# caumente/multi_task_breast_cancer

Hardware: AMD Instinct MI355X
Metric: training images/sec (1-ch 256x256, U-Net++ MT) (higher is better)
Workload: dtype bf16; 1 GPU; MTUNetPlusPlus seg+cls deep-supervision step (Dice+Focal, alpha=0.5, Adam eps 1e-4), per-GPU batch 32, 1x256x256, bf16 MFMA operands (3x3 convs, ConvT) and 16-bit stored conv outputs / activations; fp32 accumulation, gradient sums, statistics, losses, parameters and optimizer, random-init weights (BASELINE.json configs[1]); global_batch=32, parallelism=dp1

## Files before the change

include/mtbc.h:

```cpp
#ifndef MTBC_H
#define MTBC_H

#include <stddef.h>
#include <stdint.h>

#ifdef __cplusplus
extern "C" {
#endif

#define MTBC_VERSION 203
#define MTBC_MAX_SEGS 6
#define MTBC_STEM_MAX_CIN 5

enum {
    MTBC_OK = 0,
    MTBC_E_BADSHAPE = -1,
    MTBC_E_BADARG = -2,
    MTBC_E_WORKSPACE = -3,
    MTBC_E_LAUNCH = -4,
    MTBC_E_UNSUPPORTED = -5
};

int mtbc_version(void);
const char* mtbc_strerror(int code);
// ... 186 lines not shown
    float* y;
    const float* dy;
    float* dx;       int64_t dx_batch_stride;
    int32_t accumulate_dx;
    float* dw;       float* dbias;
    int32_t accumulate_dw;
    void* workspace; size_t workspace_bytes;
    int32_t x_layout;
    int32_t x_type;
} mtbc_conv1x1_args;

size_t mtbc_conv1x1_wgrad_workspace(const mtbc_conv1x1_args* a);
int mtbc_conv1x1_fwd(const mtbc_conv1x1_args* a, void* stream);
int mtbc_conv1x1_dgrad(const mtbc_conv1x1_args* a, void* stream);
int mtbc_conv1x1_wgrad(const mtbc_conv1x1_args* a, void* stream);

typedef struct {
    int32_t N, C, H, W;
    const float* x;  float* y;
    const float* dy; float* dx;
} mtbc_gap_args;
int mtbc_gap_fwd(const mtbc_gap_args* a, void* stream);
int mtbc_gap_bwd(const mtbc_gap_args* a, void* stream);

typedef struct {
    int32_t N, In, Out, relu;
    const float* x; const float* w; const float* bias; float* y;
    const float* dy; float* dx;
    float* dw; float* dbias; int32_t accumulate_dw;
    void* workspace; size_t workspace_bytes;
// ... 219 lines not shown
```

multi_task_breast_cancer_amd/_lib.py:

```python
from __future__ import annotations

import ctypes as C
import os
from typing import Optional

_HERE = os.path.dirname(os.path.abspath(__file__))
LIB_PATH = os.environ.get("MTBC_LIB") or os.path.join(_HERE, "libmtbc_hip.so")

MAX_SEGS = 6
STEM_MAX_CIN = 5
c_float_p = C.POINTER(C.c_float)


class MtbcError(RuntimeError):
    pass


LAYOUT_PLANAR, LAYOUT_C8 = 0, 1


class Seg(C.Structure):
    _fields_ = [("ptr", C.c_void_p), ("batch_stride", C.c_int64), ("channels", C.c_int32), ("accumulate", C.c_int32)]


# ... 225 lines not shown
    _fields_ = [("w", C.c_void_p), ("packed", C.c_void_p), ("Cin", C.c_int32), ("Cout", C.c_int32),
                ("kind", C.c_int32), ("compute", C.c_int32)]


class WViewDesc(C.Structure):
    _fields_ = [("w", C.c_void_p), ("dst", C.c_void_p), ("Cout", C.c_int32), ("Cin", C.c_int32), ("ci_off", C.c_int32),
                ("ci_cnt", C.c_int32), ("mode", C.c_int32), ("k_off", C.c_int32), ("K", C.c_int32)]


EXPORTS = [
    "mtbc_version", "mtbc_strerror", "mtbc_arch",
    "mtbc_conv3x3_packed_elems", "mtbc_conv3x3_packed_dgrad_elems", "mtbc_conv3x3_pack_fwd",
    "mtbc_conv3x3_pack_dgrad", "mtbc_conv3x3_packed_lp_elems", "mtbc_conv3x3_pack_lp", "mtbc_conv3x3_pack_many", "mtbc_c8_pack", "mtbc_c8_unpack", "mtbc_c8_pack16", "mtbc_conv3x3_weight_view", "mtbc_conv3x3_weight_view_many", "mtbc_augment_flip_rotate", "mtbc_convT_head_combine", "mtbc_convT_head_expand", "mtbc_conv3x3_wgrad_workspace", "mtbc_conv3x3_wgrad_sync_bytes", "mtbc_conv3x3_stats_slots", "mtbc_conv3x3_kernel_name", "mtbc_conv3x3_fwd", "mtbc_conv3x3_dgrad",
    "mtbc_conv3x3_wgrad", "mtbc_instnorm_fwd_workspace", "mtbc_instnorm_coop_state_bytes", "mtbc_instnorm_coop_error_offset", "mtbc_instnorm_c8_supported", "mtbc_instnorm_bwd_team", "mtbc_instnorm_dparam_many", "mtbc_instnorm_kernel_name", "mtbc_instnorm_lrelu_fwd", "mtbc_instnorm_lrelu_bwd", "mtbc_maxpool2_fwd",
    "mtbc_maxpool2_bwd", "mtbc_convT_wgrad_workspace", "mtbc_convT_fwd_c8_supported", "mtbc_convT_fwd", "mtbc_convT_dgrad", "mtbc_convT_wgrad",
    "mtbc_conv1x1_wgrad_workspace", "mtbc_conv1x1_fwd", "mtbc_conv1x1_dgrad", "mtbc_conv1x1_wgrad",
    "mtbc_gap_fwd", "mtbc_gap_bwd", "mtbc_linear_fwd", "mtbc_linear_bwd", "mtbc_dice_fwd", "mtbc_dice_bwd",
    "mtbc_focal_fwd_bwd", "mtbc_loss_mix", "mtbc_loss_scale_begin", "mtbc_loss_scale_check",
    "mtbc_loss_scale_update_host", "mtbc_loss_scale_begin_host", "mtbc_optim_step", "mtbc_optim_dynamic", "mtbc_loss_scale_optim", "mtbc_optim_step_host",
    "mtbc_dice_counts", "mtbc_program_run",
    "mtbc_program_run_ms", "mtbc_event_create", "mtbc_event_destroy",
    "mtbc_seg_metrics_workspace_size", "mtbc_seg_metrics", "mtbc_batch_assemble", "mtbc_train_metrics",
    "mtbc_eval_metrics",
]

ABI_VERSION = 203
_lib: Optional[C.CDLL] = None


def load() -> C.CDLL:
    global _lib
# ... 60 lines not shown
                      ("mtbc_conv1x1_wgrad", Conv1x1Args), ("mtbc_gap_fwd", GapArgs), ("mtbc_gap_bwd", GapArgs),
                      ("mtbc_linear_fwd", LinearArgs), ("mtbc_linear_bwd", LinearArgs),
                      ("mtbc_dice_fwd", DiceArgs), ("mtbc_dice_bwd", DiceArgs), ("mtbc_focal_fwd_bwd", FocalArgs)):
        getattr(lib, name).restype = C.c_int
        getattr(lib, name).argtypes = [C.POINTER(typ), C.c_void_p]
    lib.mtbc_instnorm_coop_state_bytes.restype = C.c_size_t
    lib.mtbc_instnorm_coop_state_bytes.argtypes = []
    lib.mtbc_instnorm_coop_error_offset.restype = C.c_size_t
    lib.mtbc_instnorm_coop_error_offset.argtypes = []
    lib.mtbc_instnorm_bwd_team.restype = C.c_int32
    lib.mtbc_instnorm_bwd_team.argtypes = [C.POINTER(InstNormArgs)]
    lib.mtbc_instnorm_dparam_many.restype = C.c_int
    lib.mtbc_instnorm_dparam_many.argtypes = [C.POINTER(DparamDesc), C.c_int32, C.c_void_p]
    lib.mtbc_instnorm_c8_supported.restype = C.c_int
    lib.mtbc_instnorm_c8_supported.argtypes = [C.POINTER(InstNormArgs), C.c_int32]
    lib.mtbc_convT_fwd_c8_supported.restype = C.c_int
    lib.mtbc_convT_fwd_c8_supported.argtypes = [C.POINTER(ConvTArgs)]
    lib.mtbc_loss_mix.restype = C.c_int
    lib.mtbc_loss_mix.argtypes = [C.c_void_p, C.c_void_p, C.c_float, C.c_void_p, C.c_void_p]
    lib.mtbc_dice_counts.restype = C.c_int
    lib.mtbc_dice_counts.argtypes = [C.c_void_p, C.c_void_p, C.c_int64, C.c_void_p, C.c_void_p]
    for name in ("mtbc_loss_scale_begin", "mtbc_loss_scale_check"):
        getattr(lib, name).restype = C.c_int
        getattr(lib, name).argtypes = [C.POINTER(LossScaleArgs), C.c_void_p]
    for name in ("mtbc_loss_scale_update_host", "mtbc_loss_scale_begin_host"):
        getattr(lib, name).restype = C.c_int
        getattr(lib, name).argtypes = [C.POINTER(LossScaleArgs)]
    lib.mtbc_optim_step.restype = C.c_int
    lib.mtbc_optim_step.argtypes = [C.POINTER(OptimArgs), C.c_void_p]
    lib.mtbc_optim_dynamic.restype = C.c_int
# ... 43 lines not shown
```

multi_task_breast_cancer_amd/csrc/common.h:

```cpp
#pragma once
#include <hip/hip_runtime.h>
#include <stdint.h>
#include <stdlib.h>
#include "../../include/mtbc.h"

#define MTBC_WAVE 64

typedef float f32x4 __attribute__((ext_vector_type(4)));

#define MTBC_CHECK_LAUNCH()                                   \
    do {                                                      \
        hipError_t e__ = hipGetLastError();                   \
        if (e__ != hipSuccess) return MTBC_E_LAUNCH;          \
    } while (0)

#ifdef MTBC_PROBES
#include <stdlib.h>
static inline int mtbc_probe_int(const char* name, int dflt) { const char* v = getenv(name); return v ? atoi(v) : dflt; }
static inline bool mtbc_probe_set(const char* name) { return getenv(name) != nullptr; }
#define MTBC_DBG_BIT(p, bit) ((p).dbg & (bit))
#else
#define mtbc_probe_int(name, dflt) (dflt)
#define mtbc_probe_set(name) (false)
#define MTBC_DBG_BIT(p, bit) (0)
// ... 113 lines not shown
    NK_STATS_FIN, NK_APPLY_FWD, NK_BSTATS_FIN, NK_APPLY_BWD,
    NK_R1_FIN, NK_DPARAM,
    NK_FWD_REG, NK_CHUNK_STATS, NK_CHUNK_APPLY, NK_FWD_STREAM, NK_BWD, NK_BWD_REG
};
struct NormLaunch { int k; int t[6]; int threads; int T, rounds; };
struct NormChoice {
    static constexpr int MAX = 4;
    int n; NormLaunch l[MAX];
    void add(int k, int t0 = 0, int t1 = 0, int t2 = 0, int t3 = 0, int t4 = 0, int t5 = 0) { if (n == MAX) abort(); l[n++] = NormLaunch{k, {t0, t1, t2, t3, t4, t5}, 0, 0, 0}; }
    void add(const NormLaunch& k) { if (n == MAX) abort(); l[n++] = k; }
    NormLaunch& last() { return l[n - 1]; }
};
extern "C" int mtbc_i_instnorm_fwd_c8(const mtbc_instnorm_args* a, hipStream_t st, NormChoice* query);
extern "C" int mtbc_i_instnorm_bwd_c8(const mtbc_instnorm_args* a, float* part, hipStream_t st, NormChoice* query);
extern "C" int mtbc_i_instnorm_bwd_c8_team(const mtbc_instnorm_args* a);
int mtbc_i_maxpool_c8_fwd(const mtbc_maxpool_args* a, hipStream_t st);
int mtbc_i_maxpool_c8_bwd(const mtbc_maxpool_args* a, hipStream_t st);
int mtbc_i_conv1x1_c8_fwd(const mtbc_conv1x1_args* a, hipStream_t st);
size_t mtbc_i_conv1x1_c8_wgrad_workspace(const mtbc_conv1x1_args* a);
int mtbc_i_conv1x1_c8_wgrad(const mtbc_conv1x1_args* a, hipStream_t st);
int mtbc_i_splitk_reduce(const float* partial, float* out, int nsplit, size_t elems, int accumulate, hipStream_t st);
int mtbc_i_splitk_reduce2(const float* partial, float* out, float* out2, int nsplit, size_t elems1, size_t elems2, int accumulate, hipStream_t st);
bool mtbc_i_convT2_fwd_ok(const mtbc_convT_args* a);
int mtbc_i_convT2_fwd(const mtbc_convT_args* a, hipStream_t st);
bool mtbc_i_convT2_fwd_c8_ok(const mtbc_convT_args* a);
int mtbc_i_convT2_fwd_c8(const mtbc_convT_args* a, hipStream_t st);
bool mtbc_i_convT2_fwd_lp_c8_ok(const mtbc_convT_args* a);
int mtbc_i_convT2_fwd_lp_c8(const mtbc_convT_args* a, hipStream_t st);
bool mtbc_i_convT2_dgrad_ok(const mtbc_convT_args* a);
bool mtbc_i_convT2_wgrad_ok(const mtbc_convT_args* a);
// ... 8 lines not shown
```

multi_task_breast_cancer_amd/csrc/norm_coop.hip:

```cpp
#include "common.h"
#include <stddef.h>
#include <type_traits>

namespace {

constexpr int CO_THREADS = 512, CO_WAVES = CO_THREADS / 64;
constexpr int CO_MAXT = 128, CO_NV = 16;
constexpr unsigned CO_SPIN_MAX = 1u << 26;
constexpr size_t CO_MAILBOX_OFF = 256;
constexpr int CO_MAX_TEAMS = 1024;
constexpr size_t CO_TEAM_WORDS = 2 * CO_MAXT * CO_NV;
struct CoopHdr { unsigned epoch, done, err, pad; };

struct CoP {
    int N, C, HW, G8, T, items, nteams, f16;
    float eps, slope;
    const float* z; const float* gamma; const float* beta;
    float* y; long long ybs;
    unsigned short* y8;
    float* mean; float* rstd;
    const float* dy; long long dybs;
    unsigned short* dz8;
    float* part;
    float* part3;
// ... 560 lines not shown
#pragma unroll
            for (int c = 0; c < 8; ++c) yb[(size_t)c * p.HW + px] = v[c];
        }
        if (yh) {
            if (k == 1) {
#pragma unroll
                for (int c = 0; c < 8; ++c) {
                    const unsigned lo = (okeep[c >> 1] >> (16 * (c & 1))) & 0xffffu, hi = (o[c >> 1] >> (16 * (c & 1))) & 0xffffu;
                    *reinterpret_cast<unsigned*>(yh + (size_t)c * p.HW + px - 1) = lo | (hi << 16);
                }
            } else okeep = o;
        }
    }
}

__global__ void in_bstats_finalize_kernel(const float* __restrict__ part, int slots, int C, int HW, float* __restrict__ m12,
                                          float* __restrict__ dparam_part, int planes) {
    const int plane = blockIdx.x * (blockDim.x >> 6) + (threadIdx.x >> 6), lane = threadIdx.x & 63;
    if (plane >= planes) return;
    const int n = plane / C, c = plane % C;
    const float* q = part + ((size_t)n * slots * C + c) * 2;
    double s1 = 0.0, s2 = 0.0;
    for (int t = lane; t < slots; t += 64) { const float2 v = *reinterpret_cast<const float2*>(q + (size_t)t * C * 2); s1 += (double)v.x; s2 += (double)v.y; }
    s1 = wave_sum_d(s1); s2 = wave_sum_d(s2);
    if (lane == 0) {
        m12[2 * plane] = (float)(s1 / (double)HW); m12[2 * plane + 1] = (float)(s2 / (double)HW);
        if (dparam_part) { dparam_part[3 * plane] = (float)s1; dparam_part[3 * plane + 1] = (float)s2; dparam_part[3 * plane + 2] = 0.f; }
    }
}
template <bool F16, bool ZF16>
// ... 245 lines not shown
        pl = plan_team<false>(p.items, p.HW, var_of(a), a->coop_reserve_cus);
        if (!pl.ok) return MTBC_E_UNSUPPORTED;
        choose_c8(&ch, false, p.HW, p.items, var_of(a), &pl);
    }
    if (query) { for (int i = 0; i < ch.n; ++i) query->add(ch.l[i]); return MTBC_OK; }
    for (int i = 0; i < ch.n; ++i) {
        const NormLaunch& k = ch.l[i];
        if (k.k == NK_STATS_FIN) hipLaunchKernelGGL(in_stats_finalize_kernel, dim3(cdiv(planes, 4)), dim3(256), 0, st, a->stats_partial, a->stats_slots, a->C, p.HW, a->eps, a->mean, a->rstd, planes);
        else if (k.k == NK_APPLY_FWD) launch_apply_fwd(k, g, st, p, a->stats_partial, a->stats_slots);
        else launch_chosen_c8<false>(k, p, pl, st);
        MTBC_CHECK_LAUNCH();
    }
    return MTBC_OK;
}

int mtbc_i_instnorm_bwd_c8_team(const mtbc_instnorm_args* a) {
    if (!a || a->N <= 0 || a->C <= 0 || a->C % 8) return 0;
    if (a->H * a->W <= SOLO_MAX_HW) return 1;
    const CoPlan pl = plan_team<true>(a->N * (a->C / 8), a->H * a->W, var_of(a), a->coop_reserve_cus);
    return pl.ok ? pl.T : 0;
}
int mtbc_i_instnorm_bwd_c8(const mtbc_instnorm_args* a, float* part, hipStream_t st, NormChoice* query) {
    CoP p; int rc = fill_coop(a, &p); if (rc) return rc;
    if ((!p.z && !p.z8) || (!p.dy && !p.r1 && !p.pg) || !p.dz8 || !p.mean || !p.rstd || (reinterpret_cast<uintptr_t>(p.dz8) & 15)) return MTBC_E_BADARG;
    if (!p.dy && a->dy_layout == MTBC_LAYOUT_C8) return MTBC_E_BADARG;
    if ((p.r1 || p.pg) && a->stats_partial) return MTBC_E_UNSUPPORTED;
    if (a->dy_layout == MTBC_LAYOUT_C8) {
        if ((reinterpret_cast<uintptr_t>(a->dy) & 15) || a->dy_batch_stride % 8 || a->n_dy_extra < 0 || a->n_dy_extra > 1) return MTBC_E_BADARG;
        p.dy8 = reinterpret_cast<const unsigned short*>(a->dy); p.dy8bs = a->dy_batch_stride; p.dy = nullptr;
        if (a->n_dy_extra == 1) { if (!a->dy_extra[0]) return MTBC_E_BADARG; p.dyx = a->dy_extra[0]; }
// ... 47 lines not shown
```

multi_task_breast_cancer_amd/csrc/program.hip:

```cpp
#include "common.h"

extern "C" {

int mtbc_version(void) { return MTBC_VERSION; }
const char* mtbc_arch(void) { return "gfx950"; }

const char* mtbc_strerror(int code) {
    switch (code) {
        case MTBC_OK: return "ok";
        case MTBC_E_BADSHAPE: return "bad shape";
        case MTBC_E_BADARG: return "bad argument (null or misaligned pointer)";
        case MTBC_E_WORKSPACE: return "workspace missing or too small";
        case MTBC_E_LAUNCH: return "kernel launch failed";
        case MTBC_E_UNSUPPORTED: return "unsupported configuration";
        default: return "unknown error";
    }
}

static inline bool is_pack(int32_t k) { return k == MTBC_OP_CONV3_PACK_FWD || k == MTBC_OP_CONV3_PACK_DGRAD || k == MTBC_OP_CONV3_PACK_LP; }

int mtbc_event_create(void** event) {
    if (!event) return MTBC_E_BADARG;
    hipEvent_t e;
    if (hipEventCreateWithFlags(&e, hipEventDisableTiming) != hipSuccess) return MTBC_E_LAUNCH;
// ... 66 lines not shown
        if (o->kind == MTBC_OP_IN_DPARAM) {
            mtbc_dparam_desc d[64];
            int32_t n = 0;
            while (n < 64 && i + n < first + count && ops[i + n].kind == MTBC_OP_IN_DPARAM) { d[n] = ops[i + n].u.dparam; ++n; }
            rc = mtbc_instnorm_dparam_many(d, n, stream);
            if (rc != MTBC_OK) { if (failed_index) *failed_index = i; return rc; }
            i += n - 1;
            continue;
        }
        if (o->kind == MTBC_OP_CONVT_WGRAD && i + 1 < first + count && ops[i + 1].kind == MTBC_OP_CONVT_DGRAD) {
            bool fused = false;
            rc = mtbc_i_convT_bwd_pair(&o->u.convT, &ops[i + 1].u.convT, stream, &fused);
            if (rc != MTBC_OK) { if (failed_index) *failed_index = i; return rc; }
            if (fused) { ++i; continue; }
        }
        switch (o->kind) {
            case MTBC_OP_CONV3_FWD: rc = mtbc_conv3x3_fwd(&o->u.conv3, stream); break;
            case MTBC_OP_CONV3_DGRAD: rc = mtbc_conv3x3_dgrad(&o->u.conv3, stream); break;
            case MTBC_OP_CONV3_WGRAD: rc = mtbc_conv3x3_wgrad(&o->u.conv3, stream); break;
            case MTBC_OP_CONV3_PACK_FWD: rc = mtbc_conv3x3_pack_fwd(o->u.pack.w, o->u.pack.packed, o->u.pack.Cin, o->u.pack.Cout, stream); break;
            case MTBC_OP_CONV3_PACK_DGRAD: rc = mtbc_conv3x3_pack_dgrad(o->u.pack.w, o->u.pack.packed, o->u.pack.Cin, o->u.pack.Cout, stream); break;
            case MTBC_OP_HEAD_COMBINE: rc = mtbc_convT_head_combine(&o->u.head, stream); break;
            case MTBC_OP_HEAD_EXPAND: rc = mtbc_convT_head_expand(&o->u.head, stream); break;
            case MTBC_OP_CONV3_WVIEW: rc = mtbc_conv3x3_weight_view(o->u.wview.w, o->u.wview.dst, o->u.wview.Cout, o->u.wview.Cin, o->u.wview.ci_off, o->u.wview.ci_cnt, o->u.wview.mode, o->u.wview.k_off, o->u.wview.K, stream); break;
            case MTBC_OP_C8_PACK16: rc = mtbc_c8_pack16(o->u.c8pack.src, o->u.c8pack.src_batch_stride, o->u.c8pack.dst, o->u.c8pack.N, o->u.c8pack.C, o->u.c8pack.HW, stream); break;
            case MTBC_OP_C8_PACK: rc = mtbc_c8_pack(o->u.c8pack.src, o->u.c8pack.src_batch_stride, o->u.c8pack.dst, o->u.c8pack.N, o->u.c8pack.C, o->u.c8pack.HW, o->u.c8pack.compute, stream); break;
            case MTBC_OP_CONV3_PACK_LP: rc = mtbc_conv3x3_pack_lp(o->u.pack.w, o->u.pack.packed, o->u.pack.Cin, o->u.pack.Cout, o->u.pack.dgrad, o->u.pack.compute, stream); break;
            case MTBC_OP_IN_FWD: rc = mtbc_instnorm_lrelu_fwd(&o->u.inorm, stream); break;
            case MTBC_OP_IN_BWD: rc = mtbc_instnorm_lrelu_bwd(&o->u.inorm, stream); break;
            case MTBC_OP_POOL_FWD: rc = mtbc_maxpool2_fwd(&o->u.pool, stream); break;
// ... 32 lines not shown
```

multi_task_breast_cancer_amd/engine.py:

```python
from __future__ import annotations

import ctypes as C
from dataclasses import dataclass, field
from typing import Callable, Dict, List, Optional, Sequence, Tuple

import torch

from . import _lib as L


from . import switches as _sw

_sw.refuse_removed()
_NO_COOP = _sw.flag("MTBC_NO_COOP")
_NO_GATHER = _sw.flag("MTBC_NO_GATHER")
_NO_Z16 = _sw.flag("MTBC_NO_Z16")
_Z_BF16 = _sw.flag("MTBC_Z_BF16")
_NO_STEM_MC = _sw.flag("MTBC_NO_STEM_MC")
_DA16 = _sw.flag("MTBC_DA16")
_COOP_MIN_FWD, _COOP_MIN_BWD = 16384, 65536
_IN_KERNEL_SPLITK = False
_DPARAM_BATCH = 12


# ... 123 lines not shown
                 grad_view: Callable[[str], torch.Tensor], slots: Dict[str, ParamSlot], force_direct: bool = False,
                 compute: int = 0, coop_reserve_cus: int = 0, coop_state: Optional[Callable[[], torch.Tensor]] = None):
        self.dev = device
        self._shared_coop = coop_state
        self.coop_reserve_cus = int(coop_reserve_cus)
        self.compute = int(compute)
        self.N = N
        self.pv, self.gv, self.slots = param_view, grad_view, slots
        self.force_direct = 1 if force_direct else 0
        self.cells: List[_Cell] = []
        self.keep: list = []
        self.fwd_ops: List[L.Op] = []
        self.pack_ops: List[L.Op] = []
        self.wview_ops: List[L.Op] = []
        self.bwd_emitters: List[Callable[[], None]] = []
        self.bwd_ops: List[L.Op] = []
        self.loss_ops: List[L.Op] = []
        self.ws_bytes = 0
        self.ws_users: List[Tuple[L.Op, str]] = []
        self._pending_dparams: List[Tuple[L.Op, tuple]] = []
        self._sync_users: List[L.Op] = []
        self._sync_bytes = 0
        self._stat_users: List[Tuple[L.Op, str]] = []
        self._stat_bytes = 0
        self.arena_bytes = 0
        self._tag = 0
        self.acts: Dict[str, Act] = {}
        self.lib = L.load()
        for s in slots.values():
            s.grad_written = False
# ... 656 lines not shown
            a.dwT, a.dbT = self.gv(wTname).data_ptr(), self.gv(bTname).data_ptr()
            a.dw1, a.db1 = self.gv(w1name).data_ptr(), self.gv(b1name).data_ptr()
            self.bwd_ops.append(op)
            if x.needs_grad:
                op = base()
                op.kind = L.OP_CONVT_DGRAD
                a = op.u.convT
                a.dy, a.dy_batch_stride = dy.data_ptr(), y.bstride
                gx, acc = self.grad_slot(x)
                a.dx, a.dx_batch_stride, a.accumulate_dx = gx.data_ptr(), x.bstride, acc
                self.bwd_ops.append(op)

        self.bwd_emitters.append(emit_bwd)
        return y

    def conv1x1(self, x: Act, cout: int, wname: str, bname: str, out_name: str) -> Act:
        assert x.N == self.N, f"{x.name}: only conv cells and max-pools are planned over a batch-concatenated (2N) tensor"
        w = self.pv(wname)
        assert tuple(w.shape) == (cout, x.C, 1, 1), (wname, tuple(w.shape))
        x.readers += 1
        y = self.new_act(out_name, cout, x.H, x.W)
        c8 = self._c8_small_ok(x) and cout <= 8
        x8 = self.c8_of(x) if c8 else None

        def base() -> L.Op:
            op = _mk(0)
            a = op.u.conv1
            a.N, a.H, a.W, a.Cin, a.Cout = self.N, x.H, x.W, x.C, cout
            if c8:
                a.x, a.x_batch_stride, a.x_layout, a.x_type = x8.data_ptr(), x.bstride, L.LAYOUT_C8, self.compute
            else:
# ... 21 lines not shown
            a.dy = dy.data_ptr()
            a.accumulate_dw = self._mark_param(wname)
            self._mark_param(bname)
            a.dw, a.dbias = self.gv(wname).data_ptr(), self.gv(bname).data_ptr()
            self._need_ws(op, "conv1", self.lib.mtbc_conv1x1_wgrad_workspace(C.byref(a)))
            self.bwd_ops.append(op)
            if x.needs_grad:
                op = base()
                op.kind = L.OP_CONV1_DGRAD
                a = op.u.conv1
                a.dy = dy.data_ptr()
                gx, acc = self.grad_slot(x)
                a.dx, a.dx_batch_stride, a.accumulate_dx = gx.data_ptr(), x.bstride, acc
                self.bwd_ops.append(op)

        self.bwd_emitters.append(emit_bwd)
        return y

    def gap(self, x: Act, out_name: str) -> Act:
        assert x.N == self.N, f"{x.name}: only conv cells and max-pools are planned over a batch-concatenated (2N) tensor"
        x.readers += 1
        y = Act(out_name, self.alloc(self.N, x.C, 1, 1))

        def base() -> L.Op:
            op = _mk(0)
            a = op.u.gap
            a.N, a.C, a.H, a.W = self.N, x.C, x.H, x.W
            a.x, a.y = self._rd(x), y.data.data_ptr()
            return op

        op = base()
        op.kind = L.OP_GAP_FWD
# ... 93 lines not shown
        op = _mk(L.OP_FOCAL)
        a = op.u.focal
        a.N, a.C, a.alpha, a.gamma = N, logits.C, 1.0, (0.0 if binary else float(cls_gamma))
        a.x, a.target, a.weight = logits.data.data_ptr(), onehot.data_ptr(), _ptr(focal_weight)
        a.loss, a.dx, a.gscale = self.focal_loss.data_ptr(), self.grad_of(logits).data_ptr(), (1.0 - alpha) * loss_scale
        a.gscale_dev = self.grad_weight.data_ptr()
        logits.grad_written = True
        self.loss_ops.append(op)
        op = _mk(L.OP_LOSS_MIX)
        op.u.mix.seg = self.dice_loss.data_ptr() + 4 * nh
        op.u.mix.cls, op.u.mix.alpha, op.u.mix.out4 = self.focal_loss.data_ptr(), alpha, self.loss_out.data_ptr()
        self.loss_ops.append(op)
        self.keep += [mask, onehot] + ([focal_weight] if focal_weight is not None else [])

    def emit_backward(self) -> None:
        for em in reversed(self.bwd_emitters):
            em()
        self.flush_dparams()

    def _narrow_activations(self) -> None:
        if not self.compute:
            return
        for a in self.acts.values():
            hw = a.H * a.W
            if a.p16_users:
                if a.planar_used:
                    for op in a.p16_users:
                        op.u.convT.x = a.data.data_ptr()
                else:
                    y16 = self.alloc(a.N, a.C, a.H, a.W, dtype=torch.int16)
# ... 43 lines not shown
```

multi_task_breast_cancer_amd/nets.py:

```python
from __future__ import annotations

import os

from typing import Callable, Dict, List, Optional, Sequence, Tuple

import torch
import torch.nn as nn

from . import _lib as L
from . import switches as _sw
from .engine import Act, ParamSlot, StepPlan

NNUNET_WIDTHS = (32, 64, 128, 256, 320)
UNETPP_FEATURES = (24, 48, 96, 192, 384, 24)


def _draw_conv(cin: int, cout: int, k: int, bias: bool):
    m = nn.Conv2d(cin, cout, kernel_size=k, padding=k // 2, bias=bias)
    return m.weight.detach(), (m.bias.detach() if bias else None)


def _draw_convT(cin: int, cout: int, k: int):
    m = nn.ConvTranspose2d(cin, cout, kernel_size=k, stride=k)
    return m.weight.detach(), m.bias.detach()
# ... 108 lines not shown
    enc, t = [], x
    for i in range(5):
        e = level([t], w[i], w[i], f"encoder{i + 1}")
        enc.append(e)
        t = plan.maxpool(e, f"pool{i + 1}")
    bott = level([t], w[4], w[4], "bottleneck")
    up5 = plan.convT(bott, w[4], 2, "upsample5.weight", "upsample5.bias", "up5")
    dec_out = {5: w[3], 4: w[2], 3: w[1], 2: w[0], 1: w[0] // 2}
    dec_mid = {5: w[3], 4: w[2], 3: w[1], 2: w[0], 1: w[0]}
    dec, d, up = {}, None, up5
    for i in (5, 4, 3, 2, 1):
        if i != 5:
            up = plan.convT(d, w[i - 1], 2, f"upsample{i}.weight", f"upsample{i}.bias", f"up{i}")
        d = level([enc[i - 1], up], dec_mid[i], dec_out[i], f"decoder{i}")
        dec[i] = d
    pe5 = cell([enc[4]], w[4], "process_encoder_5")
    pd5 = cell([dec[5]], w[4], "process_decoder_5")
    feat = cell([pe5, up5, pd5], 512, "classifier.0")
    g = plan.gap(feat, "gap")
    h = plan.linear(g, 256, "classifier.3.weight", "classifier.3.bias", True, "fc1")
    n_cls = plan.pv("classifier.5.weight").shape[0]
    logits = plan.linear(h, n_cls, "classifier.5.weight", "classifier.5.bias", False, "logits")
    regions = plan.pv("output1.weight").shape[0]
    if _sw.flag("MTBC_NOFUSE_HEADS"):
        o4 = plan.conv1x1(plan.convT(dec[4], w[2], 8, "output4.0.weight", "output4.0.bias", "o4up"), regions,
                          "output4.1.weight", "output4.1.bias", "output4")
        o3 = plan.conv1x1(plan.convT(dec[3], w[1], 4, "output3.0.weight", "output3.0.bias", "o3up"), regions,
                          "output3.1.weight", "output3.1.bias", "output3")
        o2 = plan.conv1x1(plan.convT(dec[2], w[0], 2, "output2.0.weight", "output2.0.bias", "o2up"), regions,
                          "output2.1.weight", "output2.1.bias", "output2")
    else:
        o4 = plan.convT_head(dec[4], w[2], 8, "output4.0.weight", "output4.0.bias", "output4.1.weight", "output4.1.bias", "output4")
        o3 = plan.convT_head(dec[3], w[1], 4, "output3.0.weight", "output3.0.bias", "output3.1.weight", "output3.1.bias", "output3")
        o2 = plan.convT_head(dec[2], w[0], 2, "output2.0.weight", "output2.0.bias", "output2.1.weight", "output2.1.bias", "output2")
    o1 = plan.conv1x1(dec[1], regions, "output1.weight", "output1.bias", "output1")
    return logits, [o4, o3, o2, o1]


def _graph_unetpp(plan: StepPlan, x: Act):
    f = UNETPP_FEATURES

    def convolution(inputs, cout, name):
        return plan.conv_cell(inputs, cout, f"{name}.conv.weight", f"{name}.conv.bias", f"{name}.adn.N.weight",
                              f"{name}.adn.N.bias", 0.1, name)

    def two_conv(inputs, cout, name):
        return convolution([convolution(inputs, cout, f"{name}.conv_0")], cout, f"{name}.conv_1")

    def down(t, cout, name, tag=""):
        return two_conv([plan.maxpool(t, f"{name}.pool{tag}")], cout, f"{name}.convs")

    def upcat(t, skips, cout, name, halves=True):
        up_c = t.C // 2 if halves else t.C
        up = plan.convT(t, up_c, 2, f"{name}.upsample.deconv.weight", f"{name}.upsample.deconv.bias", f"{name}.up")
        return two_conv(list(skips) + [up], cout, f"{name}.convs")

    x00 = two_conv([x], f[0], "conv_0_0")
    x10 = down(x00, f[1], "conv_1_0")
    x01 = upcat(x10, [x00], f[0], "upcat_0_1", halves=False)
    x20 = down(x10, f[2], "conv_2_0")
    x11 = upcat(x20, [x10], f[1], "upcat_1_1")
    x02 = upcat(x11, [x00, x01], f[0], "upcat_0_2", halves=False)
    x30 = down(x20, f[3], "conv_3_0")
    x21 = upcat(x30, [x20], f[2], "upcat_2_1")
    x12 = upcat(x21, [x10, x11], f[1], "upcat_1_2")
    x03 = upcat(x12, [x00, x01, x02], f[0], "upcat_0_3", halves=False)
    pl3_in, (p30, p31) = plan.batch_pair("process_level_3.in", f[3], x30.H // 2, x30.W // 2)
    x40 = two_conv([plan.maxpool(x30, "conv_4_0.pool", out=p30)], f[4], "conv_4_0.convs")
    x31 = upcat(x40, [x30], f[3], "upcat_3_1")
    x22 = upcat(x31, [x20, x21], f[2], "upcat_2_2")
    x13 = upcat(x22, [x10, x11, x12], f[1], "upcat_1_3")
    x04 = upcat(x13, [x00, x01, x02, x03], f[5], "upcat_0_4", halves=False)
    regions = plan.pv("final_conv_0_1.weight").shape[0]
    outs = [plan.conv1x1(t, regions, f"final_conv_0_{j}.weight", f"final_conv_0_{j}.bias", f"final_conv_0_{j}")
            for j, t in ((1, x01), (2, x02), (3, x03), (4, x04))]
    plan.maxpool(x31, "process_level_3.poolb", out=p31)
    pa, pb = plan.split_batch(two_conv([pl3_in], f[4], "process_level_3.convs"))
    feat = two_conv([pa, x40, pb], 512, "classifier.0")
    g = plan.gap(feat, "gap")
    h = plan.linear(g, 256, "classifier.3.weight", "classifier.3.bias", True, "fc1")
    n_cls = plan.pv("classifier.5.weight").shape[0]
    logits = plan.linear(h, n_cls, "classifier.5.weight", "classifier.5.bias", False, "logits")
    return logits, outs


class _Node(nn.Module):
    """Bare container used to give parameters the reference's dotted names."""


class CompiledStep:
# ... 216 lines not shown
```

multi_task_breast_cancer_amd/switches.py:

```python
from __future__ import annotations

import os
from typing import Dict, List

PLAN_SWITCHES: Dict[str, tuple] = {
    "MTBC_NO_COOP": ("0", "InstanceNorm by one-plane workgroups (fp32 conv outputs) + pack instead of the channel-group / cooperative kernels: "
                          "the fallback when their teams cannot be co-resident (the cooperative error message names it)",
                     "tests/test_model_gpu.py::test_16bit_mfma_modes_match_their_emulation[...-no_coop-40]"),
    "MTBC_NO_GATHER": ("0", "every 3x3 conv back-propagates into all its inputs (fan-in by read-modify-write) instead of one gathered launch per dense-skip tensor",
                       "tests/test_model_gpu.py::test_16bit_mfma_modes_match_their_emulation[...-no_gather]"),
    "MTBC_NO_Z16": ("0", "16-bit modes keep the conv outputs z as fp32 planes (InstanceNorm reads 4 bytes per element in both directions): the storage arm of the quality sweeps",
                    "tests/test_model_gpu.py::test_16bit_mfma_modes_match_their_emulation[...-no_z16]"),
    "MTBC_Z_BF16": ("0", "bf16 mode stores the conv outputs as bf16 instead of fp16 (same bytes, 8 instead of 11 significant bits)",
                    "tests/test_model_gpu.py::test_16bit_mfma_modes_match_their_emulation[...-z_bf16]"),
    "MTBC_DA16": ("0", "the gradient a conv-cell activation gets from its 3x3 consumers is written by ONE gathered launch as a 16-bit channel-blocked tensor (fp32 sum in the MFMA "
                       "accumulators, one RNE) instead of fp32 planar fan-in: -0.36 ms per step.  Default in round 3 on the easy task's evidence (-0.010 +- 0.025 pt); OFF again since "
                       "round 4: on the task that can fail it ends at the same Dice (-0.012 +- 0.042 pt against fp32, 10 paired seeds) but reaches the plateau LATER -- mid-run "
                       "-5.6 +- 2.9 pt against fp32 where the fp32-gradient plan is at -0.5 +- 1.4 and tracks the fp32 runs seed by seed (profiles/r04_quality_hard.md)",
                  "tests/test_model_gpu.py::test_16bit_mfma_modes_match_their_emulation[...-da16]"),
    "MTBC_NOFUSE_HEADS": ("0", "MTnnUNet deep-supervision heads as ConvT + 1x1 (the reference's two layers) instead of one combined ConvT",
                          "tests/test_model_gpu.py::test_mtnnunet_two_layer_heads_match_the_fused_heads_and_the_oracle"),
    "MTBC_GRAPH": ("0", "trainer.FusedTrainStep (single process) captures each compiled step -- weight images, forward, losses, backward, Adam -- into ONE hipGraph at its third call "
                        "and replays it from then on: the host issues a step in 0.1 ms instead of 8.4 (profiles/r04_graph_replay.txt); the GPU time is the same, the results are the same bits "
                        "(the optimizer's per-step scalars travel through device memory, mtbc_optim_args.dynamic)",
# ... 5 lines not shown
    "MTBC_NO_STEM_MC": ("0", "a first conv with intensity channels (data.augmentation: Cin 2 .. 5) takes the launches it took before the multi-channel stem kernels: "
                             "conv3x3_direct_kernel, an fp32 conv output under the one-plane InstanceNorm, the small-Cin (Cin = 5: the direct) weight gradient from fp32 dz -- "
                             "the A arm of tools/stem_cost.py",
                        "tests/test_stem_multichannel_gpu.py::test_whole_model_against_the_emulation[...-no_stem_mc]"),
    "MTBC_COOP_RESERVE_CUS": ("64", "CUs kept out of the cooperative InstanceNorm grids under data parallel",
                              "tests/test_coop_safety_gpu.py::test_cooperative_step_beside_a_cu_hogging_kernel"),
}
REMOVED = ("MTBC_NO_C8", "MTBC_NO_CT_LP", "MTBC_COOP_MIN_FWD", "MTBC_COOP_MIN_BWD", "MTBC_NO_P16", "MTBC_FANIN", "MTBC_NO_C8_SMALL_OPS", "MTBC_NO_X16",
           "MTBC_NO_G16", "MTBC_NO_EPI_STATS", "MTBC_EPI_BSTATS", "MTBC_NO_R1", "MTBC_NO_POOLFOLD", "MTBC_SPLIT_FANIN", "MTBC_NO_STEM16",
           "MTBC_NO_DEFER_DPARAM", "MTBC_DPARAM_BATCH", "MTBC_NO_POOLFWD_FOLD", "MTBC_BWD_OVERLAP", "MTBC_BWD_OVERLAP_MAX_HW",
           "MTBC_NO_DA16")
RESULT_ALTERING = ("MTBC_DBG", "MTBC_NOACC", "MTBC_LOWP", "MTBC_LP_MT", "MTBC_RING", "MTBC_NODMA", "MTBC_C8_BLOCKS_PER_CU",
                   "MTBC_WGRAD_LP1", "MTBC_CT_WG_TASKS", "MTBC_IN_BWD_STREAM", "MTBC_CONVT_GENERIC", "MTBC_C8_NW", "MTBC_C8_RING",
                   "MTBC_CT_DEPTH", "MTBC_CT_WG_CT", "MTBC_CT_WG_XCD", "MTBC_CT_DGRAD_DIRECT", "MTBC_WGRAD_C8W", "MTBC_C8W_BPC", "MTBC_C8W_DEPTH", "MTBC_C8W_HACK",
                   "MTBC_WGRAD_PACK24", "MTBC_WGRAD_C8I", "MTBC_WG_NS8", "MTBC_WG_TS", "MTBC_C8_TS", "MTBC_RING_TS", "MTBC_INB_TS",
                   "MTBC_CT_UNFUSED", "MTBC_CT_FUSE_ALL")


def get(name: str) -> str:
    return os.environ.get(name, PLAN_SWITCHES[name][0])


def flag(name: str) -> bool:
    v = get(name)
    return v not in ("", "0")


def active() -> Dict[str, str]:
    return {k: v for k, v in sorted(os.environ.items()) if k.startswith("MTBC_")}


# ... 17 lines not shown
```

Baseline: 3017 images/sec.

## Fuse InstanceNorm-LeakyReLU apply with the following 1x1 segmentation head

Adds a kernel that applies InstanceNorm and LeakyReLU to the C8-layout activation and, in the same pass, computes the single-output 1x1 head conv from the rounded 16-bit outputs. The program runner pairs an IN forward op with a directly following conv1x1 forward op when the pair is supported. The net builders are reordered so that each head conv is emitted right after the InstanceNorm of its input (U-Net++ heads after x01/x02/x03, MT U-Net output1), and the heads' backward emission is held back and released later so backward order stays the same. This removes a separate read of the full-resolution activation and one launch per head, at the cost of a serial per-pixel channel reduction and a different forward schedule.

```diff
diff --git a/include/mtbc.h b/include/mtbc.h
--- a/include/mtbc.h
+++ b/include/mtbc.h
@@ -224,6 +224,8 @@
 int mtbc_conv1x1_fwd(const mtbc_conv1x1_args* a, void* stream);
 int mtbc_conv1x1_dgrad(const mtbc_conv1x1_args* a, void* stream);
 int mtbc_conv1x1_wgrad(const mtbc_conv1x1_args* a, void* stream);
+#define MTBC_IN_HEAD_MAX_C 64
+int32_t mtbc_instnorm_head_pair_supported(const mtbc_instnorm_args* a, const mtbc_conv1x1_args* h);
 
 typedef struct {
     int32_t N, C, H, W;
diff --git a/multi_task_breast_cancer_amd/_lib.py b/multi_task_breast_cancer_amd/_lib.py
--- a/multi_task_breast_cancer_amd/_lib.py
+++ b/multi_task_breast_cancer_amd/_lib.py
@@ -263,7 +263,7 @@
     "mtbc_conv3x3_pack_dgrad", "mtbc_conv3x3_packed_lp_elems", "mtbc_conv3x3_pack_lp", "mtbc_conv3x3_pack_many", "mtbc_c8_pack", "mtbc_c8_unpack", "mtbc_c8_pack16", "mtbc_conv3x3_weight_view", "mtbc_conv3x3_weight_view_many", "mtbc_augment_flip_rotate", "mtbc_convT_head_combine", "mtbc_convT_head_expand", "mtbc_conv3x3_wgrad_workspace", "mtbc_conv3x3_wgrad_sync_bytes", "mtbc_conv3x3_stats_slots", "mtbc_conv3x3_kernel_name", "mtbc_conv3x3_fwd", "mtbc_conv3x3_dgrad",
     "mtbc_conv3x3_wgrad", "mtbc_instnorm_fwd_workspace", "mtbc_instnorm_coop_state_bytes", "mtbc_instnorm_coop_error_offset", "mtbc_instnorm_c8_supported", "mtbc_instnorm_bwd_team", "mtbc_instnorm_dparam_many", "mtbc_instnorm_kernel_name", "mtbc_instnorm_lrelu_fwd", "mtbc_instnorm_lrelu_bwd", "mtbc_maxpool2_fwd",
     "mtbc_maxpool2_bwd", "mtbc_convT_wgrad_workspace", "mtbc_convT_fwd_c8_supported", "mtbc_convT_fwd", "mtbc_convT_dgrad", "mtbc_convT_wgrad",
-    "mtbc_conv1x1_wgrad_workspace", "mtbc_conv1x1_fwd", "mtbc_conv1x1_dgrad", "mtbc_conv1x1_wgrad",
+    "mtbc_conv1x1_wgrad_workspace", "mtbc_conv1x1_fwd", "mtbc_conv1x1_dgrad", "mtbc_conv1x1_wgrad", "mtbc_instnorm_head_pair_supported",
     "mtbc_gap_fwd", "mtbc_gap_bwd", "mtbc_linear_fwd", "mtbc_linear_bwd", "mtbc_dice_fwd", "mtbc_dice_bwd",
     "mtbc_focal_fwd_bwd", "mtbc_loss_mix", "mtbc_loss_scale_begin", "mtbc_loss_scale_check",
     "mtbc_loss_scale_update_host", "mtbc_loss_scale_begin_host", "mtbc_optim_step", "mtbc_optim_dynamic", "mtbc_loss_scale_optim", "mtbc_optim_step_host",
@@ -354,6 +354,9 @@
     lib.mtbc_instnorm_dparam_many.argtypes = [C.POINTER(DparamDesc), C.c_int32, C.c_void_p]
     lib.mtbc_instnorm_c8_supported.restype = C.c_int
     lib.mtbc_instnorm_c8_supported.argtypes = [C.POINTER(InstNormArgs), C.c_int32]
+    if hasattr(lib, "mtbc_instnorm_head_pair_supported"):
+        lib.mtbc_instnorm_head_pair_supported.restype = C.c_int32
+        lib.mtbc_instnorm_head_pair_supported.argtypes = [C.POINTER(InstNormArgs), C.POINTER(Conv1x1Args)]
     lib.mtbc_convT_fwd_c8_supported.restype = C.c_int
     lib.mtbc_convT_fwd_c8_supported.argtypes = [C.POINTER(ConvTArgs)]
     lib.mtbc_loss_mix.restype = C.c_int
diff --git a/multi_task_breast_cancer_amd/csrc/common.h b/multi_task_breast_cancer_amd/csrc/common.h
--- a/multi_task_breast_cancer_amd/csrc/common.h
+++ b/multi_task_breast_cancer_amd/csrc/common.h
@@ -151,6 +151,7 @@
 extern "C" int mtbc_i_instnorm_fwd_c8(const mtbc_instnorm_args* a, hipStream_t st, NormChoice* query);
 extern "C" int mtbc_i_instnorm_bwd_c8(const mtbc_instnorm_args* a, float* part, hipStream_t st, NormChoice* query);
 extern "C" int mtbc_i_instnorm_bwd_c8_team(const mtbc_instnorm_args* a);
+extern "C" int mtbc_i_instnorm_head_pair(const mtbc_instnorm_args* a, const mtbc_conv1x1_args* h, void* stream, bool* fused);
 int mtbc_i_maxpool_c8_fwd(const mtbc_maxpool_args* a, hipStream_t st);
 int mtbc_i_maxpool_c8_bwd(const mtbc_maxpool_args* a, hipStream_t st);
 int mtbc_i_conv1x1_c8_fwd(const mtbc_conv1x1_args* a, hipStream_t st);
diff --git a/multi_task_breast_cancer_amd/csrc/norm_coop.hip b/multi_task_breast_cancer_amd/csrc/norm_coop.hip
--- a/multi_task_breast_cancer_amd/csrc/norm_coop.hip
+++ b/multi_task_breast_cancer_amd/csrc/norm_coop.hip
@@ -598,6 +598,96 @@
     }
 }
 
+constexpr int AH_MAX_C = MTBC_IN_HEAD_MAX_C;
+template <bool F16, bool FIN, bool ZF16>
+__global__ __launch_bounds__(AP_THREADS) void in_apply_head_fwd_c8_kernel(const CoP p, const float* __restrict__ part, const int slots,
+                                                                          const float* __restrict__ hw, const float* __restrict__ hb,
+                                                                          float* __restrict__ hy) {
+    __shared__ float cst[3][AH_MAX_C];
+    const int n = blockIdx.y;
+    if ((int)threadIdx.x < p.C) {
+        const int c = threadIdx.x;
+        const size_t pl = (size_t)n * p.C + c;
+        float mean, rstd;
+        if constexpr (FIN) {
+            const float* q = part + ((size_t)n * slots * p.C + c) * 2;
+            double ts = 0.0, tq = 0.0;
+#pragma unroll 1
+            for (int k0 = 0; k0 < 32; k0 += 8) {
+                float2 lo[8], hi[8];
+#pragma unroll
+                for (int u = 0; u < 8; ++u) {
+                    const int t = k0 + u;
+                    lo[u] = t < slots ? *reinterpret_cast<const float2*>(q + (size_t)t * p.C * 2) : make_float2(0.f, 0.f);
+                    hi[u] = t + 32 < slots ? *reinterpret_cast<const float2*>(q + (size_t)(t + 32) * p.C * 2) : make_float2(0.f, 0.f);
+                }
+#pragma unroll
+                for (int u = 0; u < 8; ++u) {
+                    double s = 0.0, qq = 0.0;
+                    s += (double)lo[u].x; qq += (double)lo[u].y;
+                    s += (double)hi[u].x; qq += (double)hi[u].y;
+                    ts += s; tq += qq;
+                }
+            }
+            const double m = ts / (double)p.HW, var = fmax(tq / (double)p.HW - m * m, 0.0);
+            mean = (float)m; rstd = (float)(1.0 / sqrt(var + (double)p.eps));
+            if (blockIdx.x == 0) { p.mean[pl] = mean; p.rstd[pl] = rstd; }
+        } else { mean = p.mean[pl]; rstd = p.rstd[pl]; }
+        cst[0][c] = mean; cst[1][c] = (p.gamma ? p.gamma[c] : 1.f) * rstd; cst[2][c] = p.beta ? p.beta[c] : 0.f;
+    }
+    __syncthreads();
+    const size_t gstride = (size_t)p.HW * 8;
+    const unsigned short* zg = p.z8 + (size_t)n * p.G8 * gstride;
+    unsigned short* ob = p.y8 + (size_t)n * p.G8 * gstride;
+    const int px0 = blockIdx.x * (AP_THREADS * AP_PPT) + (int)threadIdx.x;
+    const float b0 = hb ? hb[0] : 0.f;
+    float acc[AP_PPT];
+    co_u32x4 w[AP_PPT];
+#pragma unroll
+    for (int k = 0; k < AP_PPT; ++k) {
+        const int px = px0 + AP_THREADS * k;
+        acc[k] = b0;
+        w[k] = (co_u32x4){0u, 0u, 0u, 0u};
+        if (px < p.HW) w[k] = *reinterpret_cast<const co_u32x4*>(zg + (size_t)px * 8);
+    }
+    for (int g = 0; g < p.G8; ++g) {
+        co_u32x4 wn[AP_PPT];
+#pragma unroll
+        for (int k = 0; k < AP_PPT; ++k) {
+            const int px = px0 + AP_THREADS * k;
+            wn[k] = w[k];
+            if (g + 1 < p.G8 && px < p.HW) wn[k] = *reinterpret_cast<const co_u32x4*>(zg + (size_t)(g + 1) * gstride + (size_t)px * 8);
+        }
+        float mu[8], ga[8], be[8], hwg[8];
+#pragma unroll
+        for (int c = 0; c < 8; ++c) { mu[c] = cst[0][8 * g + c]; ga[c] = cst[1][8 * g + c]; be[c] = cst[2][8 * g + c]; hwg[c] = hw[8 * g + c]; }
+#pragma unroll
+        for (int k = 0; k < AP_PPT; ++k) {
+            const int px = px0 + AP_THREADS * k;
+            if (px >= p.HW) continue;
+            float v[8];
+            co_unpk<ZF16>(w[k], v);
+#pragma unroll
+            for (int c = 0; c < 8; ++c) { const float t = (v[c] - mu[c]) * ga[c] + be[c]; v[c] = t > 0.f ? t : t * p.slope; }
+            co_u32x4 o;
+#pragma unroll
+            for (int h = 0; h < 4; ++h) o[h] = co_pk<F16>(v[2 * h], v[2 * h + 1]);
+            *reinterpret_cast<co_u32x4*>(ob + (size_t)g * gstride + (size_t)px * 8) = o;
+            float r[8];
+            co_unpk<F16>(o, r);
+#pragma unroll
+            for (int e = 0; e < 8; ++e) acc[k] = fmaf(hwg[e], r[e], acc[k]);
+        }
+#pragma unroll
+        for (int k = 0; k < AP_PPT; ++k) w[k] = wn[k];
+    }
+#pragma unroll
+    for (int k = 0; k < AP_PPT; ++k) {
+        const int px = px0 + AP_THREADS * k;
+        if (px < p.HW) hy[(size_t)n * p.HW + px] = acc[k];
+    }
+}
+
 __global__ void in_bstats_finalize_kernel(const float* __restrict__ part, int slots, int C, int HW, float* __restrict__ m12,
                                           float* __restrict__ dparam_part, int planes) {
     const int plane = blockIdx.x * (blockDim.x >> 6) + (threadIdx.x >> 6), lane = threadIdx.x & 63;
@@ -873,6 +963,44 @@
     return MTBC_OK;
 }
 
+int32_t mtbc_instnorm_head_pair_supported(const mtbc_instnorm_args* a, const mtbc_conv1x1_args* h) {
+    if (!a || !h) return 0;
+    CoP p;
+    if (fill_coop(a, &p) != MTBC_OK) return 0;
+    if (!a->stats_partial || a->stats_slots <= 0 || !p.z8 || !p.y8 || !p.mean || !p.rstd || (reinterpret_cast<uintptr_t>(p.y8) & 15)) return 0;
+    if (a->pool_y8 || a->pool_arg || a->y || a->y16) return 0;
+    if (a->C > AH_MAX_C) return 0;
+    if (h->Cout != 1 || h->Cin != a->C || h->N != a->N || h->H != a->H || h->W != a->W) return 0;
+    if (h->x_layout != MTBC_LAYOUT_C8 || h->x_type != a->out16_type) return 0;
+    if (reinterpret_cast<const void*>(h->x) != a->y8 || h->x_batch_stride != (int64_t)a->C * a->H * a->W) return 0;
+    if (!h->w || !h->y || ((a->H * a->W) & 3)) return 0;
+    return 1;
+}
+
+int mtbc_i_instnorm_head_pair(const mtbc_instnorm_args* a, const mtbc_conv1x1_args* h, void* stream, bool* fused) {
+    *fused = false;
+    static const bool unfused = mtbc_probe_set("MTBC_IN_HEAD_UNFUSED");
+    if (unfused || !mtbc_instnorm_head_pair_supported(a, h)) return MTBC_OK;
+    CoP p;
+    if (fill_coop(a, &p) != MTBC_OK) return MTBC_OK;
+    hipStream_t st = (hipStream_t)stream;
+    *fused = true;
+    const int planes = a->N * a->C;
+    const bool fin = a->stats_slots <= 64, zf16 = p.f16 || p.zf16;
+    if (!fin) {
+        hipLaunchKernelGGL(in_stats_finalize_kernel, dim3(cdiv(planes, 4)), dim3(256), 0, st, a->stats_partial, a->stats_slots, a->C, p.HW, a->eps, a->mean, a->rstd, planes);
+        MTBC_CHECK_LAUNCH();
+    }
+    const dim3 g(cdiv(p.HW, AP_THREADS * AP_PPT), a->N);
+#define MTBC_AH(F16_, FIN_, ZF_) hipLaunchKernelGGL((in_apply_head_fwd_c8_kernel<F16_, FIN_, ZF_>), g, dim3(AP_THREADS), 0, st, p, a->stats_partial, a->stats_slots, h->w, h->bias, h->y)
+#define MTBC_AHT(FIN_) do { if (p.f16) MTBC_AH(true, FIN_, true); else if (zf16) MTBC_AH(false, FIN_, true); else MTBC_AH(false, FIN_, false); } while (0)
+    if (fin) MTBC_AHT(true); else MTBC_AHT(false);
+#undef MTBC_AHT
+#undef MTBC_AH
+    MTBC_CHECK_LAUNCH();
+    return MTBC_OK;
+}
+
 int mtbc_i_instnorm_bwd_c8_team(const mtbc_instnorm_args* a) {
     if (!a || a->N <= 0 || a->C <= 0 || a->C % 8) return 0;
     if (a->H * a->W <= SOLO_MAX_HW) return 1;
diff --git a/multi_task_breast_cancer_amd/csrc/program.hip b/multi_task_breast_cancer_amd/csrc/program.hip
--- a/multi_task_breast_cancer_amd/csrc/program.hip
+++ b/multi_task_breast_cancer_amd/csrc/program.hip
@@ -104,6 +104,12 @@
             if (rc != MTBC_OK) { if (failed_index) *failed_index = i; return rc; }
             if (fused) { ++i; continue; }
         }
+        if (o->kind == MTBC_OP_IN_FWD && i + 1 < first + count && ops[i + 1].kind == MTBC_OP_CONV1_FWD) {
+            bool fused = false;
+            rc = mtbc_i_instnorm_head_pair(&o->u.inorm, &ops[i + 1].u.conv1, stream, &fused);
+            if (rc != MTBC_OK) { if (failed_index) *failed_index = i; return rc; }
+            if (fused) { ++i; continue; }
+        }
         switch (o->kind) {
             case MTBC_OP_CONV3_FWD: rc = mtbc_conv3x3_fwd(&o->u.conv3, stream); break;
             case MTBC_OP_CONV3_DGRAD: rc = mtbc_conv3x3_dgrad(&o->u.conv3, stream); break;
diff --git a/multi_task_breast_cancer_amd/engine.py b/multi_task_breast_cancer_amd/engine.py
--- a/multi_task_breast_cancer_amd/engine.py
+++ b/multi_task_breast_cancer_amd/engine.py
@@ -161,6 +161,7 @@
         self.pack_ops: List[L.Op] = []
         self.wview_ops: List[L.Op] = []
         self.bwd_emitters: List[Callable[[], None]] = []
+        self._held_bwd: List[Callable[[], None]] = []
         self.bwd_ops: List[L.Op] = []
         self.loss_ops: List[L.Op] = []
         self.ws_bytes = 0
@@ -847,7 +848,7 @@
         self.bwd_emitters.append(emit_bwd)
         return y
 
-    def conv1x1(self, x: Act, cout: int, wname: str, bname: str, out_name: str) -> Act:
+    def conv1x1(self, x: Act, cout: int, wname: str, bname: str, out_name: str, hold_backward: bool = False) -> Act:
         assert x.N == self.N, f"{x.name}: only conv cells and max-pools are planned over a batch-concatenated (2N) tensor"
         w = self.pv(wname)
         assert tuple(w.shape) == (cout, x.C, 1, 1), (wname, tuple(w.shape))
@@ -899,8 +900,12 @@
                 a.dx, a.dx_batch_stride, a.accumulate_dx = gx.data_ptr(), x.bstride, acc
                 self.bwd_ops.append(op)
 
-        self.bwd_emitters.append(emit_bwd)
+        (self._held_bwd if hold_backward else self.bwd_emitters).append(emit_bwd)
         return y
+
+    def release_held_backward(self) -> None:
+        self.bwd_emitters += self._held_bwd
+        self._held_bwd = []
 
     def gap(self, x: Act, out_name: str) -> Act:
         assert x.N == self.N, f"{x.name}: only conv cells and max-pools are planned over a batch-concatenated (2N) tensor"
@@ -1024,6 +1029,7 @@
         self.keep += [mask, onehot] + ([focal_weight] if focal_weight is not None else [])
 
     def emit_backward(self) -> None:
+        assert not self._held_bwd, "conv1x1(hold_backward=True) without release_held_backward()"
         for em in reversed(self.bwd_emitters):
             em()
         self.flush_dparams()
diff --git a/multi_task_breast_cancer_amd/nets.py b/multi_task_breast_cancer_amd/nets.py
--- a/multi_task_breast_cancer_amd/nets.py
+++ b/multi_task_breast_cancer_amd/nets.py
@@ -146,6 +146,8 @@
             up = plan.convT(d, w[i - 1], 2, f"upsample{i}.weight", f"upsample{i}.bias", f"up{i}")
         d = level([enc[i - 1], up], dec_mid[i], dec_out[i], f"decoder{i}")
         dec[i] = d
+    regions = plan.pv("output1.weight").shape[0]
+    o1 = plan.conv1x1(dec[1], regions, "output1.weight", "output1.bias", "output1", hold_backward=True)
     pe5 = cell([enc[4]], w[4], "process_encoder_5")
     pd5 = cell([dec[5]], w[4], "process_decoder_5")
     feat = cell([pe5, up5, pd5], 512, "classifier.0")
@@ -153,7 +155,6 @@
     h = plan.linear(g, 256, "classifier.3.weight", "classifier.3.bias", True, "fc1")
     n_cls = plan.pv("classifier.5.weight").shape[0]
     logits = plan.linear(h, n_cls, "classifier.5.weight", "classifier.5.bias", False, "logits")
-    regions = plan.pv("output1.weight").shape[0]
     if _sw.flag("MTBC_NOFUSE_HEADS"):
         o4 = plan.conv1x1(plan.convT(dec[4], w[2], 8, "output4.0.weight", "output4.0.bias", "o4up"), regions,
                           "output4.1.weight", "output4.1.bias", "output4")
@@ -165,7 +166,7 @@
         o4 = plan.convT_head(dec[4], w[2], 8, "output4.0.weight", "output4.0.bias", "output4.1.weight", "output4.1.bias", "output4")
         o3 = plan.convT_head(dec[3], w[1], 4, "output3.0.weight", "output3.0.bias", "output3.1.weight", "output3.1.bias", "output3")
         o2 = plan.convT_head(dec[2], w[0], 2, "output2.0.weight", "output2.0.bias", "output2.1.weight", "output2.1.bias", "output2")
-    o1 = plan.conv1x1(dec[1], regions, "output1.weight", "output1.bias", "output1")
+    plan.release_held_backward()
     return logits, [o4, o3, o2, o1]
 
 
@@ -187,25 +188,32 @@
         up = plan.convT(t, up_c, 2, f"{name}.upsample.deconv.weight", f"{name}.upsample.deconv.bias", f"{name}.up")
         return two_conv(list(skips) + [up], cout, f"{name}.convs")
 
+    regions = plan.pv("final_conv_0_1.weight").shape[0]
+
+    def head(t, j):
+        return plan.conv1x1(t, regions, f"final_conv_0_{j}.weight", f"final_conv_0_{j}.bias", f"final_conv_0_{j}", hold_backward=True)
+
     x00 = two_conv([x], f[0], "conv_0_0")
     x10 = down(x00, f[1], "conv_1_0")
     x01 = upcat(x10, [x00], f[0], "upcat_0_1", halves=False)
+    o1 = head(x01, 1)
     x20 = down(x10, f[2], "conv_2_0")
     x11 = upcat(x20, [x10], f[1], "upcat_1_1")
     x02 = upcat(x11, [x00, x01], f[0], "upcat_0_2", halves=False)
+    o2 = head(x02, 2)
     x30 = down(x20, f[3], "conv_3_0")
     x21 = upcat(x30, [x20], f[2], "upcat_2_1")
     x12 = upcat(x21, [x10, x11], f[1], "upcat_1_2")
     x03 = upcat(x12, [x00, x01, x02], f[0], "upcat_0_3", halves=False)
+    o3 = head(x03, 3)
     pl3_in, (p30, p31) = plan.batch_pair("process_level_3.in", f[3], x30.H // 2, x30.W // 2)
     x40 = two_conv([plan.maxpool(x30, "conv_4_0.pool", out=p30)], f[4], "conv_4_0.convs")
     x31 = upcat(x40, [x30], f[3], "upcat_3_1")
     x22 = upcat(x31, [x20, x21], f[2], "upcat_2_2")
     x13 = upcat(x22, [x10, x11, x12], f[1], "upcat_1_3")
     x04 = upcat(x13, [x00, x01, x02, x03], f[5], "upcat_0_4", halves=False)
-    regions = plan.pv("final_conv_0_1.weight").shape[0]
-    outs = [plan.conv1x1(t, regions, f"final_conv_0_{j}.weight", f"final_conv_0_{j}.bias", f"final_conv_0_{j}")
-            for j, t in ((1, x01), (2, x02), (3, x03), (4, x04))]
+    outs = [o1, o2, o3, head(x04, 4)]
+    plan.release_held_backward()
     plan.maxpool(x31, "process_level_3.poolb", out=p31)
     pa, pb = plan.split_batch(two_conv([pl3_in], f[4], "process_level_3.convs"))
     feat = two_conv([pa, x40, pb], 512, "classifier.0")
diff --git a/multi_task_breast_cancer_amd/switches.py b/multi_task_breast_cancer_amd/switches.py
--- a/multi_task_breast_cancer_amd/switches.py
+++ b/multi_task_breast_cancer_amd/switches.py
@@ -43,7 +43,7 @@
                    "MTBC_WGRAD_LP1", "MTBC_CT_WG_TASKS", "MTBC_IN_BWD_STREAM", "MTBC_CONVT_GENERIC", "MTBC_C8_NW", "MTBC_C8_RING",
                    "MTBC_CT_DEPTH", "MTBC_CT_WG_CT", "MTBC_CT_WG_XCD", "MTBC_CT_DGRAD_DIRECT", "MTBC_WGRAD_C8W", "MTBC_C8W_BPC", "MTBC_C8W_DEPTH", "MTBC_C8W_HACK",
                    "MTBC_WGRAD_PACK24", "MTBC_WGRAD_C8I", "MTBC_WG_NS8", "MTBC_WG_TS", "MTBC_C8_TS", "MTBC_RING_TS", "MTBC_INB_TS",
-                   "MTBC_CT_UNFUSED", "MTBC_CT_FUSE_ALL")
+                   "MTBC_CT_UNFUSED", "MTBC_CT_FUSE_ALL", "MTBC_IN_HEAD_UNFUSED")
 
 
 def get(name: str) -> str:
```

After: 3037 images/sec, median of 6. No clear change (+0.7%).
